# zju3dv/LoFTR

Hardware: AMD Instinct MI355X
Metric: image-pairs/sec @640x480 indoor-ds (higher is better)
Workload: dtype f32; 1 GPU; batch=8 640x480 synthetic grayscale pairs per GPU, indoor_ds dual-softmax (BASELINE configs[1]), full LoFTR.forward = ResNet-FPN backbone (HIP implicit-GEMM / patch convolutions incl. the 7x7 stem) + HIP matching path; weights=seeded random init (no checkpoint on the box), conf_matrix_materialised=True, match_type=dual_softmax, global_batch=8, parallelism=dp1 (pairs sharded; RCCL all-gather of match counts)

## Files before the change

### loftr_amd/build.py

```python
import os
import subprocess
import sys
from concurrent.futures import ThreadPoolExecutor

HERE = os.path.dirname(os.path.abspath(__file__))
CSRC = os.path.join(HERE, "csrc")
OBJ_DIR = os.path.join(CSRC, "build")
LIB_PATH = os.path.join(HERE, "libloftr_hip.so")
SOURCES = ["linear.hip", "coarse_plan.hip", "attention.hip", "transformer.hip", "coarse_match.hip", "fine.hip", "misc.hip",
           "sp_convert.hip", "conv.hip", "eval.hip", "input.hip", "comm.hip", "pose.hip", "train.hip", "train_bwd.hip", "encoder_fused.hip", "fine_fused.hip", "head_grads.hip", "encoder_bwd.hip", "fine_bwd.hip", "train_glue.hip", "bank.hip", "pose_gpu.hip", "window_head.hip", "window_head_first.hip", "geometry.hip", "geometry_gpu.hip", "absolute_pose.hip", "absolute_pose_gpu.hip", "scan.hip", "atlas.hip", "atlas_gpu.hip", "triangulate.hip", "triangulate_gpu.hip", "model_lookup.hip", "model_lookup_gpu.hip", "bundle.hip", "bundle_gpu.hip", "register.hip", "register_gpu.hip", "complete.hip", "complete_gpu.hip", "merge.hip", "merge_gpu.hip", "split.hip", "split_gpu.hip", "similarity.hip", "similarity_gpu.hip", "overlap.hip", "overlap_gpu.hip", "undistort.hip", "undistort_gpu.hip", "refine.hip", "refine_gpu.hip", "rotation.hip", "rotation_gpu.hip"]
FLAGS = ["--offload-arch=gfx950", "-O3", "-std=c++17", "-fPIC", "-Wall", "-Wno-unused-parameter"]


def _hipcc():
    for c in (os.environ.get("HIPCC"), "/opt/rocm/bin/hipcc", "hipcc"):
        if c and (os.path.isabs(c) and os.path.exists(c) or not os.path.isabs(c)):
            return c
    raise RuntimeError("hipcc not found")


def _deps_mtime():
    paths = [os.path.join(CSRC, f) for f in os.listdir(CSRC) if f.endswith((".h", ".hip"))]
    paths.append(os.path.join(os.path.dirname(HERE), "include", "loftr_hip.h"))
    return max(os.path.getmtime(p) for p in paths)


def build(force=False, verbose=True, extra_flags=(), lib_path=None, obj_dir=None):
    global LIB_PATH, OBJ_DIR
    lib_default, obj_default = LIB_PATH, OBJ_DIR
    if lib_path:
        LIB_PATH, OBJ_DIR, force = lib_path, obj_dir or (OBJ_DIR + "_variant"), True
    try:
        return _build(force, verbose, tuple(extra_flags))
    finally:
        LIB_PATH, OBJ_DIR = lib_default, obj_default


def _build(force, verbose, extra_flags):
    if not force and os.path.exists(LIB_PATH) and os.path.getmtime(LIB_PATH) >= _deps_mtime():
        return LIB_PATH
    os.makedirs(OBJ_DIR, exist_ok=True)
    hipcc = _hipcc()

    def compile_one(src):
        obj = os.path.join(OBJ_DIR, src.replace(".hip", ".o"))
        cmd = [hipcc, *FLAGS, *extra_flags, "-c", os.path.join(CSRC, src), "-o", obj]
        r = subprocess.run(cmd, capture_output=True, text=True)
        if r.returncode != 0:
            raise RuntimeError(f"hipcc failed on {src}:\n{r.stderr}")
        if verbose and r.stderr.strip():
            sys.stderr.write(r.stderr)
        return obj

    with ThreadPoolExecutor(max_workers=min(8, len(SOURCES))) as ex:
        objs = list(ex.map(compile_one, SOURCES))
    vs = os.path.join(OBJ_DIR, "exports.map")
    with open(vs, "w") as fh:
        fh.write("{ global: loftr_*; local: *; };\n")
    r = subprocess.run([hipcc, "--offload-arch=gfx950", "-shared", "-fPIC", f"-Wl,--version-script={vs}", "-o", LIB_PATH, *objs, "-ldl"],
                       capture_output=True, text=True)
    if r.returncode != 0:
        raise RuntimeError(f"link failed:\n{r.stderr}")
    if verbose:
        print(f"built {LIB_PATH} ({os.path.getsize(LIB_PATH) / 1e6:.2f} MB)")
    return LIB_PATH


if __name__ == "__main__":
    if "--variant" in sys.argv:
        i = sys.argv.index("--variant")
        name = sys.argv[i + 1]
        build(extra_flags=[a for a in sys.argv[i + 2:] if a.startswith("-")],
              lib_path=os.path.join(HERE, f"libloftr_hip_{name}.so"), obj_dir=os.path.join(CSRC, "build", f"variant_{name}"))
    else:
        build(force="--force" in sys.argv)
```

### loftr_amd/csrc/common.h

```cpp
#pragma once
#include <hip/hip_runtime.h>
#include <stdint.h>
#include <stddef.h>
#include "../../include/loftr_hip.h"

typedef float f32x16 __attribute__((ext_vector_type(16)));
typedef float f32x4 __attribute__((ext_vector_type(4)));
typedef float f32x2 __attribute__((ext_vector_type(2)));

#define LOFTR_NEG_INF (-1e9f)

#define LOFTR_CHECK_ARG(cond) do { if (!(cond)) return LOFTR_ERR_BAD_ARG; } while (0)
#define LOFTR_CHECK_LAUNCH() do { if (hipGetLastError() != hipSuccess) return LOFTR_ERR_LAUNCH; } while (0)

#ifdef __HIP_DEVICE_COMPILE__
#define LOFTR_NO_PACKED_FP32 __attribute__((target("no-packed-fp32-ops")))
#else
#define LOFTR_NO_PACKED_FP32
#endif

__host__ __device__ static inline int ceil_div(int a, int b) { return (a + b - 1) / b; }
static inline size_t align_up(size_t x, size_t a) { return (x + a - 1) / a * a; }

enum LoftrTimedKernel {
  LOFTR_T_SCORE_STATS = 0,
  LOFTR_T_SCORE_CONF = 1,
  LOFTR_T_PROJ = 2,
  LOFTR_T_LINEAR = 3,
  LOFTR_T_LINEAR_LN = 4,
  LOFTR_T_KV = 5,
  LOFTR_T_ATTN_APPLY = 6,
  LOFTR_T_ATTN_SMALL = 7,
  LOFTR_T_GATHER = 8,
  LOFTR_T_OT_STORE = 9,
  LOFTR_T_CONV = 10,
  LOFTR_T_CONV3 = 11,
  LOFTR_T_CONV3W = 12,
  LOFTR_T_ENCODER_X = 13,
  LOFTR_T_FINE_PAIR = 14,
  LOFTR_T_COUNT = 15
};
enum LoftrDebugKey {
  LOFTR_DBG_ENCODER_SCHEDULE = 0,
  LOFTR_DBG_CONV_PERSIST_CAP,
  LOFTR_DBG_WGRAD_CHUNK,
  LOFTR_DBG_REDUCE_TALL,
  LOFTR_DBG_PCT_GRID,
  LOFTR_DBG_PCT_SKIP,
  LOFTR_DBG_PCT_QUOTA,
  LOFTR_DBG_CONV_DUO,
  LOFTR_DBG_CONV_PATCH,
  LOFTR_DBG_CONV_REM,
  LOFTR_DBG_FINE_WAVES,
  LOFTR_DBG_COUNT
};
int loftr_debug_value(int key);
extern unsigned g_loftr_timing_mask;
extern int g_loftr_range_check;
void loftr_timing_mark(int id, hipStream_t st, bool end);
struct TimedLaunch {
  int id; hipStream_t st; bool on;
  TimedLaunch(int id_, hipStream_t st_) : id(id_), st(st_), on((g_loftr_timing_mask >> id_) & 1u) {
    if (on) loftr_timing_mark(id, st, false);
  }
  ~TimedLaunch() { if (on) loftr_timing_mark(id, st, true); }
};

constexpr int NUM_XCD = 8;
static inline unsigned xcd_grid(int tiles_m, int tiles_n) { return (unsigned)(NUM_XCD * ceil_div(tiles_m, NUM_XCD) * tiles_n); }
__device__ __forceinline__ bool xcd_tile(int tiles_m, int tiles_n, int& tile_m, int& tile_n) {
  const int id = blockIdx.x, xcd = id % NUM_XCD, slot = id / NUM_XCD;
  const int chunk = ceil_div(tiles_m, NUM_XCD);
  tile_n = slot % tiles_n;
  const int local = slot / tiles_n;
  tile_m = xcd * chunk + local;
  return local < chunk && tile_m < tiles_m;
}

struct WsAlloc {
  char* base; size_t cap; size_t off;
  WsAlloc(void* p, size_t bytes) : base((char*)p), cap(bytes), off(0) {}
  template <typename T> T* take(size_t n) {
    off = align_up(off, 256);
    T* r = (T*)(base + off);
    off += n * sizeof(T);
    return r;
  }
  bool ok() const { return off <= cap; }
};

__device__ __forceinline__ float wave_sum(float v) {
#pragma unroll
  for (int o = 32; o >= 1; o >>= 1) v += __shfl_xor(v, o, 64);
  return v;
}
__device__ __forceinline__ float wave_max(float v) {
#pragma unroll
  for (int o = 32; o >= 1; o >>= 1) v = fmaxf(v, __shfl_xor(v, o, 64));
  return v;
}
#define LOFTR_DPP(v_, ctrl_) __int_as_float(__builtin_amdgcn_update_dpp(0, __float_as_int(v_), ctrl_, 0xF, 0xF, true))
#define LOFTR_DPPI(v_, ctrl_) __builtin_amdgcn_update_dpp(0, v_, ctrl_, 0xF, 0xF, true)
__device__ __forceinline__ float half_sum(float v) {
  v += LOFTR_DPP(v, 0xB1);
  v += LOFTR_DPP(v, 0x4E);
  v += LOFTR_DPP(v, 0x141);
  v += LOFTR_DPP(v, 0x140);
  const auto r = __builtin_amdgcn_permlane16_swap(__float_as_int(v), __float_as_int(v), false, false);
  return __int_as_float(r[0]) + __int_as_float(r[1]);
}
__device__ __forceinline__ float half_max(float v) {
  v = fmaxf(v, LOFTR_DPP(v, 0xB1));
  v = fmaxf(v, LOFTR_DPP(v, 0x4E));
  v = fmaxf(v, LOFTR_DPP(v, 0x141));
  v = fmaxf(v, LOFTR_DPP(v, 0x140));
  const auto r = __builtin_amdgcn_permlane16_swap(__float_as_int(v), __float_as_int(v), false, false);
  return fmaxf(__int_as_float(r[0]), __int_as_float(r[1]));
}
__device__ __forceinline__ int half_min_i32(int v) {
  v = min(v, LOFTR_DPPI(v, 0xB1));
  v = min(v, LOFTR_DPPI(v, 0x4E));
  v = min(v, LOFTR_DPPI(v, 0x141));
  v = min(v, LOFTR_DPPI(v, 0x140));
  const auto r = __builtin_amdgcn_permlane16_swap(v, v, false, false);
  return min((int)r[0], (int)r[1]);
}
__device__ __forceinline__ void half_sum16(f32x16& v) {
#pragma unroll
  for (int r = 0; r < 16; ++r) v[r] += LOFTR_DPP(v[r], 0xB1);
#pragma unroll
  for (int r = 0; r < 16; ++r) v[r] += LOFTR_DPP(v[r], 0x4E);
#pragma unroll
  for (int r = 0; r < 16; ++r) v[r] += LOFTR_DPP(v[r], 0x141);
#pragma unroll
  for (int r = 0; r < 16; ++r) v[r] += LOFTR_DPP(v[r], 0x140);
#pragma unroll
  for (int r = 0; r < 16; ++r) {
    const auto q = __builtin_amdgcn_permlane16_swap(__float_as_int(v[r]), __float_as_int(v[r]), false, false);
    v[r] = __int_as_float(q[0]) + __int_as_float(q[1]);
  }
}
__device__ __forceinline__ void half_max16(f32x16& v) {
#pragma unroll
  for (int r = 0; r < 16; ++r) v[r] = fmaxf(v[r], LOFTR_DPP(v[r], 0xB1));
#pragma unroll
  for (int r = 0; r < 16; ++r) v[r] = fmaxf(v[r], LOFTR_DPP(v[r], 0x4E));
#pragma unroll
  for (int r = 0; r < 16; ++r) v[r] = fmaxf(v[r], LOFTR_DPP(v[r], 0x141));
#pragma unroll
  for (int r = 0; r < 16; ++r) v[r] = fmaxf(v[r], LOFTR_DPP(v[r], 0x140));
#pragma unroll
  for (int r = 0; r < 16; ++r) {
    const auto q = __builtin_amdgcn_permlane16_swap(__float_as_int(v[r]), __float_as_int(v[r]), false, false);
    v[r] = fmaxf(__int_as_float(q[0]), __int_as_float(q[1]));
  }
}
__device__ __forceinline__ float swap32(float v) {
  const auto r = __builtin_amdgcn_permlane32_swap(__float_as_int(v), __float_as_int(v), false, false);
  return __int_as_float((threadIdx.x & 32) ? r[0] : r[1]);
}
#define LOFTR_DPP_SWAP32(v_) swap32(v_)

__device__ __forceinline__ float elu1(float x) {
  return x > 0.f ? x + 1.f : __expf(x);
}
```

### loftr_amd/csrc/conv.hip

```cpp
#include "gemm.h"
#include "conv_prepared.h"
#include <stdlib.h>

namespace {

using CfgD = GemmCfg<256, 128, 4, 2, 3>;

struct ConvArgs {
  ASrc a;
  const sp_t* w; int K;
  const float* bias;
  const float* wscale;
  const float* x_inv;
  const sp_t* residual;
  sp_t* y_sp;
  float* y_f32;
  int M, Cout, Coutp;
  int act;
  const sp_t* up;
  int Hl, Wl;
  float sy, sx;
};

template <typename Cfg, bool FULL>
__device__ __forceinline__ void conv_epilogue(const ConvArgs& p, f32x16 (&acc)[Cfg::TM][Cfg::TN], int m0, int n0) {
  const EpiLane<Cfg> e;
  const sp_t* rs = p.residual ? p.residual + (long)m0 * p.Coutp + n0 : nullptr;
  sp_t* os = p.y_sp ? p.y_sp + (long)m0 * p.Coutp + n0 : nullptr;
  float* of = p.y_f32 ? p.y_f32 + (long)m0 * p.Cout + n0 : nullptr;
#pragma unroll
  for (int j = 0; j < Cfg::TN; ++j) {
    const int col = n0 + e.lcol + j * 32;
    const bool creal = col < p.Cout;
    const bool cpad = col < p.Coutp;
    const float b = (p.bias && creal) ? p.bias[col] : 0.f;
    const float wsc = (creal ? p.wscale[col] : 1.f) * (p.x_inv ? *p.x_inv : 1.f);
#pragma unroll
    for (int i = 0; i < Cfg::TM; ++i) {
      f32x16 v = acc[i][j] * wsc;
      if (rs) {
        uint32_t w[16];
#pragma unroll
        for (int r = 0; r < 16; ++r) {
          const int trow = e.lrow + e.rr(i, r);
          const bool ok = (FULL || m0 + trow < p.M) && cpad;
          w[r] = ok ? rs[(unsigned)(trow * p.Coutp + e.spcol + j * 32)] : 0u;
        }
#pragma unroll
        for (int r = 0; r < 16; ++r) v[r] += sp_value(w[r], e.odd);
      }
#pragma unroll
      for (int r = 0; r < 16; ++r) {
        float x = v[r] + b;
        if (p.act == 1) x = fmaxf(x, 0.f);
        if (p.act == 2) x = x > 0.f ? x : 0.01f * x;
        v[r] = creal ? x : 0.f;
      }
      if (of) {
#pragma unroll
        for (int r = 0; r < 16; ++r) {
          const int trow = e.lrow + e.rr(i, r);
          if ((FULL || m0 + trow < p.M) && creal) of[(unsigned)(trow * p.Cout + e.lcol + j * 32)] = v[r];
        }
      }
      if (os) {
        uint32_t w[16];
        sp_words16(v, e.odd, w);
#pragma unroll
        for (int r = 0; r < 16; ++r) {
          const int trow = e.lrow + e.rr(i, r);
          if ((FULL || m0 + trow < p.M) && cpad) os[(unsigned)(trow * p.Coutp + e.spcol + j * 32)] = w[r];
        }
      }
    }
  }
}

template <typename Cfg>
__device__ __forceinline__ void conv_epilogue_up(const ConvArgs& p, f32x16 (&acc)[Cfg::TM][Cfg::TN], int m0, int n0,
                                                 float* lds) {
  constexpr int LD = Cfg::BN + 4;
  static_assert(Cfg::BM * LD <= Cfg::LDS_FLOATS, "accumulator tile does not fit the operand ring");
  const EpiLane<Cfg> e;
  __syncthreads();
  const float xinv = p.x_inv ? *p.x_inv : 1.f;
#pragma unroll
  for (int j = 0; j < Cfg::TN; ++j) {
    const int col = n0 + e.lcol + j * 32;
    const float wsc = (col < p.Cout ? p.wscale[col] : 1.f) * xinv;
#pragma unroll
    for (int i = 0; i < Cfg::TM; ++i)
#pragma unroll
      for (int r = 0; r < 16; ++r) lds[(e.lrow + e.rr(i, r)) * LD + e.lcol + j * 32] = acc[i][j][r] * wsc;
  }
  __syncthreads();
  const int Wo = 2 * p.Wl, Ho = 2 * p.Hl;
  constexpr int OCTS = Cfg::BN / 8;
  for (int it = threadIdx.x; it < Cfg::BM * OCTS; it += Cfg::THREADS) {
    const int row = it / OCTS, oct = it - row * OCTS;
    const int pix = m0 + row, col0 = n0 + oct * 8;
    if (pix >= p.M || col0 >= p.Coutp) continue;
    const int t = pix / Wo, x = pix - t * Wo;
    const int bb = t / Ho, y = t - bb * Ho;
    const float fy = p.sy * (float)y, fx = p.sx * (float)x;
    const int y0 = (int)fy, x0 = (int)fx;
    const int dy = y0 < p.Hl - 1 ? p.Wl * p.Coutp : 0, dx = x0 < p.Wl - 1 ? p.Coutp : 0;
    const float ly = fy - (float)y0, lx = fx - (float)x0;
    const float hy = 1.f - ly, hx = 1.f - lx;
    const int off = sp_octet_off(col0 >> 3);
    const sp_t* s00 = p.up + (unsigned)(((bb * p.Hl + y0) * p.Wl + x0) * p.Coutp + off);
    const sp_t* src[4] = {s00, s00 + dx, s00 + dy, s00 + dy + dx};
    u32x4 hi[4], lo[4];
#pragma unroll
    for (int k = 0; k < 4; ++k) {
      hi[k] = *reinterpret_cast<const u32x4*>(src[k]);
      lo[k] = *reinterpret_cast<const u32x4*>(src[k] + 16);
    }
    float v[4][8], o[8];
#pragma unroll
    for (int k = 0; k < 4; ++k) sp_unpack8(hi[k], lo[k], v[k]);
    const f32x4 a0 = *reinterpret_cast<const f32x4*>(&lds[row * LD + oct * 8]);
    const f32x4 a1 = *reinterpret_cast<const f32x4*>(&lds[row * LD + oct * 8 + 4]);
#pragma unroll
    for (int c = 0; c < 8; ++c)
      o[c] = col0 + c < p.Cout
                 ? (c < 4 ? a0[c] : a1[c - 4]) + (hy * (hx * v[0][c] + lx * v[1][c]) + ly * (hx * v[2][c] + lx * v[3][c]))
                 : 0.f;
    u32x4 oh, ol;
    sp_pack8(o, oh, ol);
    sp_t* dst = p.y_sp + (unsigned)(pix * p.Coutp + off);
    *reinterpret_cast<u32x4*>(dst) = oh;
    *reinterpret_cast<u32x4*>(dst + 16) = ol;
  }
}

template <typename Cfg, bool UP>
__global__ __launch_bounds__(Cfg::THREADS, 2) void conv_kernel(ConvArgs p) {
  __shared__ __attribute__((aligned(16))) float lds[Cfg::LDS_FLOATS];
  int tm, tn;
  if (!xcd_tile(ceil_div(p.M, Cfg::BM), ceil_div(p.Coutp, Cfg::BN), tm, tn)) return;
  const int m0 = tm * Cfg::BM, n0 = tn * Cfg::BN;
  f32x16 acc[Cfg::TM][Cfg::TN];
  gemm_mainloop<Cfg, true>(p.a, p.w, p.K, p.M, p.Cout, p.K, m0, n0, lds, acc, p.Coutp);
  if constexpr (UP) conv_epilogue_up<Cfg>(p, acc, m0, n0, lds);
  else if (m0 + Cfg::BM <= p.M) conv_epilogue<Cfg, true>(p, acc, m0, n0);
  else conv_epilogue<Cfg, false>(p, acc, m0, n0);
}

namespace c3 {
constexpr int TY = 8, TX = 32, PW = TX + 2, PH = TY + 2, PROWS = PW * PH;
constexpr int PSLOTS = 43, PQ = 6;
constexpr int PATCH_BYTES = PSLOTS * 1024, BTILE_BYTES = 128 * 128;
constexpr int NB = 4;
constexpr int LDS_BYTES = 2 * PATCH_BYTES + NB * BTILE_BYTES + 1024;
// ... 462 lines not shown
}

template <int RT>
__global__ __launch_bounds__(256) void conv_rem_gather_kernel(const float* __restrict__ pbuf, long npix, int H, int W, int R, int c0, int Coutp,
                                                              const float* __restrict__ bias, const sp_t* __restrict__ residual, int act,
                                                              sp_t* __restrict__ y_sp) {
  const long pix = (long)blockIdx.x * 256 + threadIdx.x;
  if (pix >= npix) return;
  const int x = (int)(pix % W), y = (int)((pix / W) % H);
  float v[8];
#pragma unroll
  for (int c = 0; c < 8; ++c) v[c] = 0.f;
  const float* pp = pbuf + pix * (9 * R);
#pragma unroll
  for (int ky = 0; ky < 3; ++ky)
#pragma unroll
    for (int kx = 0; kx < 3; ++kx) {
      const int yy = y + ky - 1, xx = x + kx - 1;
      if ((unsigned)yy < (unsigned)H && (unsigned)xx < (unsigned)W) {
        const float* q = pp + ((long)(ky - 1) * W + (kx - 1)) * (9 * R) + (ky * 3 + kx) * R;
        if (RT == 4) {
          const f32x4 t = *reinterpret_cast<const f32x4*>(q);
          v[0] += t[0]; v[1] += t[1]; v[2] += t[2]; v[3] += t[3];
        } else {
#pragma unroll
          for (int c = 0; c < 7; ++c) if (c < R) v[c] += q[c];
        }
      }
    }
  sp_t* row = y_sp + pix * Coutp + c0;
  float rv[8];
#pragma unroll
  for (int c = 0; c < 8; ++c) rv[c] = 0.f;
  if (residual) {
    const sp_t* rr = residual + pix * Coutp + c0;
    const u32x4 hi = *reinterpret_cast<const u32x4*>(rr), lo = *reinterpret_cast<const u32x4*>(rr + 16);
    sp_unpack8(hi, lo, rv);
  }
  const float slope = act == 1 ? 0.f : act == 2 ? 0.01f : 1.f;
  float o[8];
#pragma unroll
  for (int c = 0; c < 8; ++c) {
    const float t = v[c] + ((bias && c < R) ? bias[c0 + c] : 0.f) + rv[c];
    o[c] = c < R ? fmaxf(t, slope * t) : 0.f;
  }
  u32x4 oh, ol;
  sp_pack8(o, oh, ol);
  const u32x4 z = {0u, 0u, 0u, 0u};
  u32x4* dst = reinterpret_cast<u32x4*>(row);
  dst[0] = oh; dst[1] = z; dst[2] = z; dst[3] = z; dst[4] = ol; dst[5] = z; dst[6] = z; dst[7] = z;
}


static int conv_prepare(const float* weight, const long* weight_strides, int Cin, int Cout, int KH, int KW,
                        const float* bn_weight, const float* bn_bias, const float* bn_mean, const float* bn_var, float bn_eps,
                        void* buf, size_t bytes, hipStream_t st) {
  LOFTR_CHECK_ARG(weight && weight_strides && buf && Cin > 0 && Cout > 0 && KH > 0 && KW > 0);
  LOFTR_CHECK_ARG((bn_weight == nullptr) == (bn_bias == nullptr) && (bn_weight == nullptr) == (bn_mean == nullptr) &&
                  (bn_weight == nullptr) == (bn_var == nullptr));
  ConvPrepared pr;
  if (!conv_prepared_layout(buf, bytes, Cin, Cout, KH, KW, pr)) return LOFTR_ERR_WORKSPACE;
  const int Cp = ceil32(Cin), K = KH * KW * Cp;
  (void)hipMemsetAsync(pr.zeros, 0, 256, st);
  hipLaunchKernelGGL(conv_rowscale_kernel, dim3(Cout), dim3(256), 0, st, weight, bn_weight, bn_bias, bn_mean, bn_var, bn_eps,
                     Cin, KH, KW, weight_strides[0], weight_strides[1], weight_strides[2], weight_strides[3], pr.bias, pr.wscale);
  hipLaunchKernelGGL(conv_prep_kernel, dim3(ceil_div(K / 32, 8), Cout), dim3(256), 0, st, weight, bn_weight, bn_bias,
                     bn_mean, bn_var, bn_eps, Cin, Cp, KH, KW, weight_strides[0], weight_strides[1], weight_strides[2],
                     weight_strides[3], pr.wsp, pr.wscale);
  LOFTR_CHECK_LAUNCH();
  return LOFTR_OK;
}

static int conv_rem_channels(int Cout, int KH, int KW, int stride) {
  return (KH == 3 && KW == 3 && stride == 1 && ceil32(Cout) == 224 && Cout - 192 >= 1 && Cout - 192 <= 7) ? Cout - 192 : 0;
}
extern "C" size_t loftr_conv_scratch_bytes(int B, int H, int W, int Cout, int KH, int KW, int stride) {
  const int R = conv_rem_channels(Cout, KH, KW, stride);
  return (R > 0 && B > 0 && H > 0 && W > 0) ? (size_t)B * H * W * 9 * R * 4 : 0;
}

static int conv_run(const uint32_t* x_sp, int B, int H, int W, int Cin, const void* prepared, size_t prepared_bytes, int Cout,
                    int KH, int KW, int stride, int pad, int act, const uint32_t* residual_sp, const uint32_t* up_sp,
                    uint32_t* y_sp, float* y_f32, void* stream, const float* x_inv = nullptr, void* scratch = nullptr, size_t scratch_bytes = 0) {
  LOFTR_CHECK_ARG(x_sp && prepared && (y_sp || y_f32) && B >= 0 && H > 0 && W > 0 && Cin > 0 && Cout > 0);
  const bool shared_gpu = (act & LOFTR_CONV_SHARED_GPU) != 0;
  act &= ~LOFTR_CONV_SHARED_GPU;
  LOFTR_CHECK_ARG(KH > 0 && KW > 0 && stride > 0 && pad >= 0 && act >= 0 && act <= 2);
  if (B == 0) return LOFTR_OK;
  hipStream_t st = (hipStream_t)stream;
  ConvGeom g;
  g.H = H; g.W = W; g.Cp = ceil32(Cin); g.KH = KH; g.KW = KW; g.stride = stride; g.pad = pad;
  g.Ho = (H + 2 * pad - KH) / stride + 1;
  g.Wo = (W + 2 * pad - KW) / stride + 1;
  if (g.Ho <= 0 || g.Wo <= 0 || H >= 32768 || W >= 32768) return LOFTR_ERR_UNSUPPORTED;
  if (up_sp && ((g.Ho & 1) || (g.Wo & 1) || KH != 1 || KW != 1 || stride != 1 || pad != 0 || !y_sp || y_f32 || residual_sp || act != 0))
    return LOFTR_ERR_UNSUPPORTED;
  const long M = (long)B * g.Ho * g.Wo;
  if (M * (long)ceil32(Cout) >= (1L << 31) || (long)B * H * W * g.Cp >= (1L << 31)) return LOFTR_ERR_UNSUPPORTED;
  const int K = KH * KW * g.Cp;
  ConvPrepared pr;
  if (!conv_prepared_layout(const_cast<void*>(prepared), prepared_bytes, Cin, Cout, KH, KW, pr)) return LOFTR_ERR_WORKSPACE;
  sp_t* wsp = pr.wsp;
  float* bias = pr.bias;
  sp_t* zeros = pr.zeros;
  g.zeros = zeros;
  ConvArgs p;
  p.a = asrc_conv(x_sp, g);
  p.w = wsp; p.K = K; p.bias = bias; p.wscale = pr.wscale; p.x_inv = x_inv; p.residual = residual_sp; p.y_sp = y_sp; p.y_f32 = y_f32;
  p.M = (int)M; p.Cout = Cout; p.Coutp = ceil32(Cout); p.act = act;
  p.up = up_sp; p.Hl = g.Ho / 2; p.Wl = g.Wo / 2;
  p.sy = g.Ho > 1 ? (float)(p.Hl - 1) / (float)(g.Ho - 1) : 0.f;
  p.sx = g.Wo > 1 ? (float)(p.Wl - 1) / (float)(g.Wo - 1) : 0.f;
  if (loftr_debug_value(LOFTR_DBG_CONV_PATCH) && KH == 3 && KW == 3 && stride == 1 && pad == 1 && !up_sp) {
    Conv3Args c;
    c.x = x_sp; c.B = B; c.H = H; c.W = W; c.Cp = g.Cp; c.Cin = Cin; c.w = wsp; c.K = K; c.bias = bias; c.wscale = pr.wscale; c.x_inv = x_inv; c.residual = residual_sp;
    c.y_sp = y_sp; c.y_f32 = y_f32; c.Cout = Cout; c.Coutp = ceil32(Cout); c.act = act; c.zeros = zeros;
    c.tiles_x = ceil_div(W, c3::TX); c.tiles_y = ceil_div(H, c3::TY); c.pbuf = nullptr;
    const bool duo = loftr_debug_value(LOFTR_DBG_CONV_DUO) != 0;
    const bool wide = duo && c.Coutp == 32 * 7;
    TimedLaunch tl(wide ? LOFTR_T_CONV3W : LOFTR_T_CONV3, st);
    if (duo && c.Coutp % 128 == 0) {
      using CF = c3d::Cfg<4, 2, 4>;
      c.tiles_y = ceil_div(H, CF::TY);
      hipLaunchKernelGGL((conv3x3_duo_kernel<CF>), dim3(xcd_grid(B * c.tiles_x * c.tiles_y, c.Coutp / 128)), dim3(256), 0, st, c);
    } else if (duo && c.Coutp == 192) {
      using CF = c3d::Cfg<6, 2, 4, 8, 2>;
      c.tiles_y = ceil_div(H, CF::TY);
      hipLaunchKernelGGL((conv3x3_duo_kernel<CF>), dim3(xcd_grid(B * c.tiles_x * c.tiles_y, 1)), dim3(512), 0, st, c);
    } else if (wide && conv_rem_channels(Cout, KH, KW, stride) > 0 && !y_f32 && loftr_debug_value(LOFTR_DBG_CONV_REM) &&
               scratch && scratch_bytes >= (size_t)B * H * W * 9 * conv_rem_channels(Cout, KH, KW, stride) * 4) {
      using CF = c3d::Cfg<6, 2, 4, 8, 2, true>;
      c.tiles_y = ceil_div(H, CF::TY);
      c.pbuf = reinterpret_cast<float*>(scratch);
      hipLaunchKernelGGL((conv3x3_duo_kernel<CF>), dim3(xcd_grid(B * c.tiles_x * c.tiles_y, 1)), dim3(512), 0, st, c);
      LOFTR_CHECK_LAUNCH();
      const long npix = (long)B * H * W;
      if (Cout - 192 == 4)
        hipLaunchKernelGGL(conv_rem_gather_kernel<4>, dim3((unsigned)((npix + 255) / 256)), dim3(256), 0, st, c.pbuf, npix, H, W, 4, 192, c.Coutp,
                           bias, residual_sp, act, y_sp);
      else
        hipLaunchKernelGGL(conv_rem_gather_kernel<0>, dim3((unsigned)((npix + 255) / 256)), dim3(256), 0, st, c.pbuf, npix, H, W, Cout - 192, 192, c.Coutp,
                           bias, residual_sp, act, y_sp);
    } else if (wide) {
      using CF = c3d::Cfg<7, 2, 4, 8, 2>;
      c.tiles_y = ceil_div(H, CF::TY);
      hipLaunchKernelGGL((conv3x3_duo_kernel<CF>), dim3(xcd_grid(B * c.tiles_x * c.tiles_y, 1)), dim3(512), 0, st, c);
    } else
      hipLaunchKernelGGL(conv3x3_kernel, dim3(shared_gpu ? xcd_grid(B * c.tiles_x * c.tiles_y, ceil_div(c.Coutp, 128))
                                                         : persistent_grid(xcd_grid(B * c.tiles_x * c.tiles_y, ceil_div(c.Coutp, 128)))),
                         dim3(512), 0, st, c);
    LOFTR_CHECK_LAUNCH();
    return LOFTR_OK;
  }
  {
    TimedLaunch tl(LOFTR_T_CONV, st);
    if (up_sp)
      hipLaunchKernelGGL((conv_kernel<CfgD, true>), dim3(xcd_grid(ceil_div(p.M, CfgD::BM), ceil_div(p.Coutp, CfgD::BN))),
                         dim3(CfgD::THREADS), 0, st, p);
    else
      hipLaunchKernelGGL((conv_kernel<CfgD, false>), dim3(xcd_grid(ceil_div(p.M, CfgD::BM), ceil_div(p.Coutp, CfgD::BN))),
                         dim3(CfgD::THREADS), 0, st, p);
  }
  LOFTR_CHECK_LAUNCH();
  return LOFTR_OK;
}

#ifdef LOFTR_CONV_PROBE
extern "C" int loftr_conv_probe_buffer(void* buf) {
  long long* b = (long long*)buf;
  return hipMemcpyToSymbol(HIP_SYMBOL(g_conv_probe), &b, sizeof(b)) == hipSuccess ? LOFTR_OK : LOFTR_ERR_LAUNCH;
}
#endif

extern "C" int loftr_conv_prepare(const float* weight, const long* weight_strides, int Cin, int Cout, int KH, int KW,
                                  const float* bn_weight, const float* bn_bias, const float* bn_mean, const float* bn_var,
                                  float bn_eps, void* prepared, size_t prepared_bytes, void* stream) {
  return conv_prepare(weight, weight_strides, Cin, Cout, KH, KW, bn_weight, bn_bias, bn_mean, bn_var, bn_eps, prepared,
                      prepared_bytes, (hipStream_t)stream);
}

extern "C" int loftr_conv_bn_act_prepared(const uint32_t* x_sp, int B, int H, int W, int Cin, const void* prepared,
                                          size_t prepared_bytes, int Cout, int KH, int KW, int stride, int pad, int act,
                                          const uint32_t* residual_sp, const uint32_t* low_sp, uint32_t* y_sp, float* y_f32,
                                          const float* x_inv_scale, void* stream) {
  return conv_run(x_sp, B, H, W, Cin, prepared, prepared_bytes, Cout, KH, KW, stride, pad, act, residual_sp, low_sp, y_sp, y_f32,
                  stream, x_inv_scale);
}

extern "C" int loftr_conv_bn_act_prepared_scratch(const uint32_t* x_sp, int B, int H, int W, int Cin, const void* prepared,
                                                  size_t prepared_bytes, int Cout, int KH, int KW, int stride, int pad, int act,
                                                  const uint32_t* residual_sp, const uint32_t* low_sp, uint32_t* y_sp, float* y_f32,
                                                  const float* x_inv_scale, void* scratch, size_t scratch_bytes, void* stream) {
  return conv_run(x_sp, B, H, W, Cin, prepared, prepared_bytes, Cout, KH, KW, stride, pad, act, residual_sp, low_sp, y_sp, y_f32,
                  stream, x_inv_scale, scratch, scratch_bytes);
}

extern "C" int loftr_conv_bn_act(const uint32_t* x_sp, int B, int H, int W, int Cin, const float* weight,
                                 const long* weight_strides, int Cout, int KH, int KW, int stride, int pad, const float* bn_weight, const float* bn_bias,
                                 const float* bn_mean, const float* bn_var, float bn_eps, int act,
                                 const uint32_t* residual_sp, uint32_t* y_sp, float* y_f32, void* ws, size_t ws_bytes,
                                 const float* x_inv_scale, void* stream) {
  LOFTR_CHECK_ARG(x_sp && (y_sp || y_f32) && B >= 0 && H > 0 && W > 0);
  if (B == 0) return LOFTR_OK;
  const int rc = conv_prepare(weight, weight_strides, Cin, Cout, KH, KW, bn_weight, bn_bias, bn_mean, bn_var, bn_eps, ws, ws_bytes,
                              (hipStream_t)stream);
  if (rc != LOFTR_OK) return rc;
  return conv_run(x_sp, B, H, W, Cin, ws, ws_bytes, Cout, KH, KW, stride, pad, act, residual_sp, nullptr, y_sp, y_f32, stream, x_inv_scale);
}

extern "C" int loftr_conv1x1_upsample_add(const uint32_t* x_sp, int B, int H, int W, int Cin, const float* weight,
                                          const long* weight_strides, int Cout, const uint32_t* low_sp, uint32_t* y_sp,
                                          void* ws, size_t ws_bytes, void* stream) {
  LOFTR_CHECK_ARG(x_sp && low_sp && y_sp && B >= 0 && H > 0 && W > 0);
  if (B == 0) return LOFTR_OK;
  const int rc = conv_prepare(weight, weight_strides, Cin, Cout, 1, 1, nullptr, nullptr, nullptr, nullptr, 0.f, ws, ws_bytes,
                              (hipStream_t)stream);
  if (rc != LOFTR_OK) return rc;
  return conv_run(x_sp, B, H, W, Cin, ws, ws_bytes, Cout, 1, 1, 1, 0, 0, nullptr, low_sp, y_sp, nullptr, stream);
}

extern "C" int loftr_stem_conv_bn_relu(const float* x, const long* x_strides, int B, int H, int W, const float* weight,
                                       const long* weight_strides, int C0, const float* bn_weight, const float* bn_bias,
                                       const float* bn_mean, const float* bn_var, float bn_eps, uint32_t* y_sp,
                                       void* stream) {
  LOFTR_CHECK_ARG(x && x_strides && weight && weight_strides && y_sp && B >= 0 && H > 0 && W > 0 && C0 > 0);
  LOFTR_CHECK_ARG((bn_weight == nullptr) == (bn_bias == nullptr) && (bn_weight == nullptr) == (bn_mean == nullptr) &&
                  (bn_weight == nullptr) == (bn_var == nullptr));
  if (C0 > 128) return LOFTR_ERR_UNSUPPORTED;
  if (B == 0) return LOFTR_OK;
  const int Ho = (H + 6 - 7) / 2 + 1, Wo = (W + 6 - 7) / 2 + 1;
  hipLaunchKernelGGL(stem_conv_kernel, dim3(ceil_div(Wo, STEM_TX), ceil_div(Ho, STEM_TY), B), dim3(256), 0,
                     (hipStream_t)stream, x, x_strides[0], x_strides[2], x_strides[3], H, W, weight, weight_strides[0],
                     weight_strides[2], weight_strides[3], bn_weight, bn_bias, bn_mean, bn_var, bn_eps, C0, Ho, Wo, y_sp);
  LOFTR_CHECK_LAUNCH();
  return LOFTR_OK;
}

extern "C" int loftr_upsample2x_add(const uint32_t* low_sp, const uint32_t* lateral_sp, uint32_t* out_sp, int B, int Hl,
                                    int Wl, int C, void* stream) {
  LOFTR_CHECK_ARG(low_sp && lateral_sp && out_sp && B >= 0 && Hl > 0 && Wl > 0 && C > 0);
  if (B == 0) return LOFTR_OK;
  const int Cp = ceil32(C);
  const long pixels = (long)B * 4 * Hl * Wl;
  if (pixels >= (1L << 31)) return LOFTR_ERR_UNSUPPORTED;
  const long nitems = pixels * (Cp / 8);
  if ((nitems + 255) / 256 >= (1L << 31)) return LOFTR_ERR_UNSUPPORTED;
  hipLaunchKernelGGL(upsample_add_kernel, dim3((unsigned)((nitems + 255) / 256)), dim3(256), 0, (hipStream_t)stream,
                     low_sp, lateral_sp, out_sp, Hl, Wl, Cp, nitems);
  LOFTR_CHECK_LAUNCH();
  return LOFTR_OK;
}

extern "C" int loftr_sp_from_f32(const float* src, uint32_t* dst_sp, long rows, int C, void* stream) {
  LOFTR_CHECK_ARG(src && dst_sp && rows >= 0 && C > 0);
  return launch_sp_convert1(src, C, dst_sp, rows, C, (hipStream_t)stream);
}

extern "C" int loftr_sp_from_f32_scaled(const float* src, uint32_t* dst_sp, long rows, int C, float* inv_scale_out, void* stream) {
  LOFTR_CHECK_ARG(src && dst_sp && inv_scale_out && rows >= 0 && C > 0);
  return launch_sp_convert1(src, C, dst_sp, rows, C, (hipStream_t)stream, inv_scale_out);
}

extern "C" int loftr_sp_to_f32(const uint32_t* src_sp, float* dst, long rows, int C, void* stream) {
  LOFTR_CHECK_ARG(src_sp && dst && rows >= 0 && C > 0);
  if (rows == 0) return LOFTR_OK;
  const int Cp = ceil32(C);
  hipLaunchKernelGGL(sp_to_f32_kernel, dim3((unsigned)rows), dim3(Cp > 256 ? 256 : Cp), 0, (hipStream_t)stream, src_sp,
                     dst, rows, C, Cp);
  LOFTR_CHECK_LAUNCH();
  return LOFTR_OK;
}
```

### loftr_amd/csrc/misc.hip

```cpp
#include "common.h"
#include <string.h>

namespace {
template <bool CL>
__global__ void pos_encode_flatten_kernel(loftr_fmap f, const float* __restrict__ pe,
                                          int pe_h, int pe_w, float* __restrict__ out, int C) {
  __shared__ float tile[32][33];
  const int H = f.H, W = f.W, HW = H * W;
  const int n = blockIdx.z, hw0 = blockIdx.x * 32, c0 = blockIdx.y * 32;
  const float* in = f.data + (long)n * f.sn;
  for (int k = threadIdx.y; k < 32; k += 8) {
    const int c = c0 + k, hw = hw0 + threadIdx.x;
    float v = 0.f;
    if (c < C && hw < HW) {
      const int y = hw / W, x = hw - y * W;
      v = pe[((long)c * pe_h + y) * pe_w + x];
      if (!CL) v += in[(long)c * f.sc + (long)y * f.sh + (long)x * f.sw];
    }
    tile[k][threadIdx.x] = v;
  }
  __syncthreads();
  for (int k = threadIdx.y; k < 32; k += 8) {
    const int hw = hw0 + k, c = c0 + threadIdx.x;
    if (hw < HW && c < C) {
      float v = tile[threadIdx.x][k];
      if (CL) { const int y = hw / W, x = hw - y * W; v += in[(long)y * f.sh + (long)x * f.sw + c]; }
      out[((long)n * HW + hw) * C + c] = v;
    }
  }
}
}

extern "C" int loftr_pos_encode_flatten(const loftr_fmap* feat, const float* pe, int pe_h, int pe_w, float* out,
                                        int N, int C, void* stream) {
  LOFTR_CHECK_ARG(feat && feat->data && pe && out && N >= 0 && C > 0 && feat->H > 0 && feat->W > 0 &&
                  feat->H <= pe_h && feat->W <= pe_w);
  if (N == 0) return LOFTR_OK;
  const dim3 grid(ceil_div(feat->H * feat->W, 32), ceil_div(C, 32), N), block(32, 8);
  if (feat->sc == 1)
    hipLaunchKernelGGL((pos_encode_flatten_kernel<true>), grid, block, 0, (hipStream_t)stream, *feat, pe, pe_h, pe_w, out, C);
  else
    hipLaunchKernelGGL((pos_encode_flatten_kernel<false>), grid, block, 0, (hipStream_t)stream, *feat, pe, pe_h, pe_w, out, C);
  LOFTR_CHECK_LAUNCH();
  return LOFTR_OK;
}

namespace {
struct DebugSwitch { const char* name; int def; int value; };
DebugSwitch g_debug[LOFTR_DBG_COUNT] = {{"encoder_schedule", 1, 1}, {"conv_persist_cap", 0, 0}, {"wgrad_chunk", 0, 0}, {"reduce_tall", 1, 1},
                                        {"pct_grid", 0, 0}, {"pct_skip", 0, 0}, {"pct_quota", 0, 0}, {"conv_duo", 1, 1}, {"conv_patch", 1, 1}, {"conv_rem", 1, 1},
                                        {"fine_waves", 0, 0}};
}
int loftr_debug_value(int key) { return (key >= 0 && key < LOFTR_DBG_COUNT) ? g_debug[key].value : 0; }
extern "C" int loftr_hip_debug_set(const char* key, int value) {
  LOFTR_CHECK_ARG(key != nullptr);
  for (auto& d : g_debug)
    if (strcmp(d.name, key) == 0) { d.value = value; return LOFTR_OK; }
  return LOFTR_ERR_BAD_ARG;
}
extern "C" int loftr_hip_debug_get(const char* key, int* value, int* default_value) {
  LOFTR_CHECK_ARG(key != nullptr && value != nullptr);
  for (auto& d : g_debug)
    if (strcmp(d.name, key) == 0) { *value = d.value; if (default_value) *default_value = d.def; return LOFTR_OK; }
  return LOFTR_ERR_BAD_ARG;
}

unsigned g_loftr_timing_mask = 0;
int g_loftr_range_check = 0;
extern "C" int loftr_hip_range_check_enable(int on) { g_loftr_range_check = on ? 1 : 0; return LOFTR_OK; }
namespace {
constexpr int T_POOL = 4096;
struct TimingSlot {
  hipEvent_t ev[T_POOL][2];
  int created, used;
  double total_ms; long long launches;
};
TimingSlot g_slots[LOFTR_T_COUNT];
const char* const T_NAMES[LOFTR_T_COUNT] = {"score_sweep_kernel<0>", "score_sweep_kernel<1>", "proj_kernel", "linear_kernel",
                                            "linear_ln_kernel", "proj_kv_kernel", "attn_apply_kernel",
                                            "attn_small_kernel", "gather_windows_kernel", "score_sweep_kernel<2>", "conv_kernel",
                                            "conv3x3_duo_kernel<Cfg<4,2,4,4,1>>", "conv3x3_duo_kernel<Cfg<7,2,4,8,2>>", "encoder_x_kernel", "fine_pair_kernel"};
void timing_drain(TimingSlot& s) {
  for (int i = 0; i < s.used; ++i) {
    float ms = 0.f;
    if (hipEventSynchronize(s.ev[i][1]) == hipSuccess && hipEventElapsedTime(&ms, s.ev[i][0], s.ev[i][1]) == hipSuccess) {
      s.total_ms += ms;
      s.launches += 1;
    }
  }
  s.used = 0;
}
}

void loftr_timing_mark(int id, hipStream_t st, bool end) {
  TimingSlot& s = g_slots[id];
  if (!end) {
    if (s.used >= T_POOL) return;
    if (s.used >= s.created) {
      if (hipEventCreate(&s.ev[s.created][0]) != hipSuccess || hipEventCreate(&s.ev[s.created][1]) != hipSuccess) return;
      s.created++;
    }
    (void)hipEventRecord(s.ev[s.used][0], st);
  } else {
    if (s.used >= s.created) return;
    (void)hipEventRecord(s.ev[s.used][1], st);
    s.used++;
  }
}

extern "C" int loftr_hip_timing_enable(unsigned mask) {
  g_loftr_timing_mask = mask & ((1u << LOFTR_T_COUNT) - 1u);
  return LOFTR_OK;
}

extern "C" int loftr_hip_timing_kernel_count(void) { return LOFTR_T_COUNT; }

extern "C" const char* loftr_hip_timing_kernel_name(int id) {
  return (id >= 0 && id < LOFTR_T_COUNT) ? T_NAMES[id] : "";
}

extern "C" int loftr_hip_timing_read(int id, double* total_ms, long long* launches, int reset) {
  LOFTR_CHECK_ARG(id >= 0 && id < LOFTR_T_COUNT && total_ms && launches);
  TimingSlot& s = g_slots[id];
  timing_drain(s);
  *total_ms = s.total_ms;
  *launches = s.launches;
  if (reset) { s.total_ms = 0.0; s.launches = 0; }
  return LOFTR_OK;
}

extern "C" int loftr_hip_abi_version(void) { return LOFTR_HIP_ABI_VERSION; }

extern "C" const char* loftr_hip_status_string(int status) {
  switch (status) {
    case LOFTR_OK: return "ok";
    case LOFTR_ERR_BAD_ARG: return "bad argument (null pointer or invalid shape)";
    case LOFTR_ERR_UNSUPPORTED: return "shape not supported by the gfx950 kernels";
    case LOFTR_ERR_WORKSPACE: return "workspace too small";
    case LOFTR_ERR_LAUNCH: return "HIP kernel launch failed";
    case LOFTR_ERR_NO_DEVICE: return "no gfx950 (MI355X) device";
    case LOFTR_ERR_COMM: return "RCCL unavailable or a communicator / collective call failed";
    case LOFTR_ERR_RANGE: return "an activation entering the split-fp16 GEMM chain is not below the fp16 maximum 65504 (or not finite)";
    default: return "unknown status";
  }
}

extern "C" int loftr_hip_device_check(void) {
  int dev = 0;
  if (hipGetDevice(&dev) != hipSuccess) return LOFTR_ERR_NO_DEVICE;
  hipDeviceProp_t prop;
  if (hipGetDeviceProperties(&prop, dev) != hipSuccess) return LOFTR_ERR_NO_DEVICE;
  return strncmp(prop.gcnArchName, "gfx950", 6) == 0 ? LOFTR_OK : LOFTR_ERR_NO_DEVICE;
}
```

Measured before the change: 478.0 image-pairs/s.

## Add pipelined split-fp16 MFMA implicit-GEMM conv path for 224-channel layers

Adds a new implicit-GEMM convolution kernel that streams activation patches and weights into LDS through direct global-to-LDS loads with a multi-stage pipeline, then runs split-fp16 32x32x16 MFMAs with pinned scheduling. It is enabled by default for convolutions without upsample or residual inputs, but the default rule only selects it for Coutp==224, choosing a wide or lean tile form depending on kernel size. It aims to replace the generic conv kernel for those layers with better overlap of loads and math, at the cost of more code paths and tuning that may not suit every shape.

```diff
diff --git a/loftr_amd/build.py b/loftr_amd/build.py
--- a/loftr_amd/build.py
+++ b/loftr_amd/build.py
@@ -8,7 +8,7 @@
 OBJ_DIR = os.path.join(CSRC, "build")
 LIB_PATH = os.path.join(HERE, "libloftr_hip.so")
 SOURCES = ["linear.hip", "coarse_plan.hip", "attention.hip", "transformer.hip", "coarse_match.hip", "fine.hip", "misc.hip",
-           "sp_convert.hip", "conv.hip", "eval.hip", "input.hip", "comm.hip", "pose.hip", "train.hip", "train_bwd.hip", "encoder_fused.hip", "fine_fused.hip", "head_grads.hip", "encoder_bwd.hip", "fine_bwd.hip", "train_glue.hip", "bank.hip", "pose_gpu.hip", "window_head.hip", "window_head_first.hip", "geometry.hip", "geometry_gpu.hip", "absolute_pose.hip", "absolute_pose_gpu.hip", "scan.hip", "atlas.hip", "atlas_gpu.hip", "triangulate.hip", "triangulate_gpu.hip", "model_lookup.hip", "model_lookup_gpu.hip", "bundle.hip", "bundle_gpu.hip", "register.hip", "register_gpu.hip", "complete.hip", "complete_gpu.hip", "merge.hip", "merge_gpu.hip", "split.hip", "split_gpu.hip", "similarity.hip", "similarity_gpu.hip", "overlap.hip", "overlap_gpu.hip", "undistort.hip", "undistort_gpu.hip", "refine.hip", "refine_gpu.hip", "rotation.hip", "rotation_gpu.hip"]
+           "sp_convert.hip", "conv.hip", "entry_gemm.hip", "eval.hip", "input.hip", "comm.hip", "pose.hip", "train.hip", "train_bwd.hip", "encoder_fused.hip", "fine_fused.hip", "head_grads.hip", "encoder_bwd.hip", "fine_bwd.hip", "train_glue.hip", "bank.hip", "pose_gpu.hip", "window_head.hip", "window_head_first.hip", "geometry.hip", "geometry_gpu.hip", "absolute_pose.hip", "absolute_pose_gpu.hip", "scan.hip", "atlas.hip", "atlas_gpu.hip", "triangulate.hip", "triangulate_gpu.hip", "model_lookup.hip", "model_lookup_gpu.hip", "bundle.hip", "bundle_gpu.hip", "register.hip", "register_gpu.hip", "complete.hip", "complete_gpu.hip", "merge.hip", "merge_gpu.hip", "split.hip", "split_gpu.hip", "similarity.hip", "similarity_gpu.hip", "overlap.hip", "overlap_gpu.hip", "undistort.hip", "undistort_gpu.hip", "refine.hip", "refine_gpu.hip", "rotation.hip", "rotation_gpu.hip"]
 FLAGS = ["--offload-arch=gfx950", "-O3", "-std=c++17", "-fPIC", "-Wall", "-Wno-unused-parameter"]
 
 
diff --git a/loftr_amd/csrc/common.h b/loftr_amd/csrc/common.h
--- a/loftr_amd/csrc/common.h
+++ b/loftr_amd/csrc/common.h
@@ -52,6 +52,7 @@
   LOFTR_DBG_CONV_PATCH,
   LOFTR_DBG_CONV_REM,
   LOFTR_DBG_FINE_WAVES,
+  LOFTR_DBG_CONV_ENTRY,
   LOFTR_DBG_COUNT
 };
 int loftr_debug_value(int key);
diff --git a/loftr_amd/csrc/conv.hip b/loftr_amd/csrc/conv.hip
--- a/loftr_amd/csrc/conv.hip
+++ b/loftr_amd/csrc/conv.hip
@@ -1,5 +1,6 @@
 #include "gemm.h"
 #include "conv_prepared.h"
+#include "entry_gemm.h"
 #include <stdlib.h>
 
 namespace {
@@ -768,6 +769,21 @@
     LOFTR_CHECK_LAUNCH();
     return LOFTR_OK;
   }
+  const int entry = loftr_debug_value(LOFTR_DBG_CONV_ENTRY);
+  if (entry && !up_sp && !residual_sp && egm::entry_gemm_takes(p.Coutp)) {
+    egm::Args e;
+    e.x = x_sp; e.H = H; e.W = W; e.Cp = g.Cp; e.Cin = Cin; e.KH = KH; e.KW = KW; e.stride = stride; e.pad = pad; e.Ho = g.Ho; e.Wo = g.Wo;
+    e.zeros = zeros; e.w = wsp; e.K = K; e.bias = bias; e.wscale = pr.wscale; e.x_inv = x_inv; e.y_sp = y_sp; e.y_f32 = y_f32;
+    e.M = p.M; e.Cout = Cout; e.Coutp = p.Coutp; e.act = act;
+    const egm::Form form = entry == 2 ? egm::FORM_LEAN : entry == 3 ? egm::FORM_WIDE : egm::entry_gemm_rule(e);
+    if (form != egm::FORM_NONE) {
+      TimedLaunch tl(LOFTR_T_CONV, st);
+      const int rc = egm::launch_entry_gemm(e, form, st);
+      if (rc != LOFTR_OK) return rc;
+      LOFTR_CHECK_LAUNCH();
+      return LOFTR_OK;
+    }
+  }
   {
     TimedLaunch tl(LOFTR_T_CONV, st);
     if (up_sp)
diff --git a/loftr_amd/csrc/entry_gemm.h b/loftr_amd/csrc/entry_gemm.h
--- /dev/null
+++ b/loftr_amd/csrc/entry_gemm.h
@@ -0,0 +1,18 @@
+#pragma once
+#include "gemm.h"
+
+namespace egm {
+struct Args {
+  const sp_t* x; int H, W, Cp, Cin;
+  int KH, KW, stride, pad, Ho, Wo;
+  const sp_t* zeros;
+  const sp_t* w; int K;
+  const float* bias; const float* wscale; const float* x_inv;
+  sp_t* y_sp; float* y_f32;
+  int M, Cout, Coutp, act;
+};
+enum Form { FORM_NONE = 0, FORM_LEAN = 1, FORM_WIDE = 2 };
+bool entry_gemm_takes(int Coutp);
+Form entry_gemm_rule(const Args& a);
+int launch_entry_gemm(const Args& a, Form form, hipStream_t st);
+}
diff --git a/loftr_amd/csrc/entry_gemm.hip b/loftr_amd/csrc/entry_gemm.hip
--- /dev/null
+++ b/loftr_amd/csrc/entry_gemm.hip
@@ -0,0 +1,290 @@
+#include "entry_gemm.h"
+
+#ifndef EGM_SETPRIO
+#define EGM_SETPRIO 0
+#endif
+#ifndef EGM_PIN
+#define EGM_PIN 1
+#endif
+
+namespace egm {
+
+template <int NT_, int RW_, int WAVES_, int WN_, int NB_>
+struct Cfg {
+  static constexpr int NT = NT_, RW = RW_, WAVES = WAVES_, WN = WN_, NB = NB_, LA = NB_ - 1;
+  static constexpr int WM = WAVES / WN, NJ = (NT + WN - 1) / WN;
+  static constexpr int BM = WM * RW * 32;
+  static constexpr int ASLOTS = BM / 16, AQ = ASLOTS / WAVES;
+  static constexpr int BSLOTS = NT * 2, BQ = (BSLOTS + WAVES - 1) / WAVES;
+  static constexpr int PER = AQ + BQ;
+  static constexpr int STAGE_BYTES = (ASLOTS + BSLOTS) * 1024;
+  static constexpr int LDS_BYTES = NB * STAGE_BYTES + 1024;
+  static constexpr int WG_PER_CU = WAVES == 4 ? 2 : 1;
+  static_assert(ASLOTS % WAVES == 0, "A slots divide evenly over the waves");
+  static_assert(LDS_BYTES * WG_PER_CU <= 160 * 1024, "LDS");
+  static_assert(RW * NJ <= 8, "128 accumulator registers");
+  static_assert(LA >= 2 && LA <= 3, "vmcnt bookkeeping below");
+  static_assert(NT - (WN - 1) * NJ >= 1, "every column split owns a tile");
+};
+
+template <int J, int NJW, int RW>
+__device__ __forceinline__ void pin_tiles() {
+  if constexpr (J + 1 < NJW) {
+    __builtin_amdgcn_sched_group_barrier(0x008, 1, 0);
+    __builtin_amdgcn_sched_group_barrier(0x100, 1, 0);
+    __builtin_amdgcn_sched_group_barrier(0x008, 1, 0);
+    __builtin_amdgcn_sched_group_barrier(0x100, 1, 0);
+    __builtin_amdgcn_sched_group_barrier(0x008, 3 * RW - 2, 0);
+    pin_tiles<J + 1, NJW, RW>();
+  } else {
+    __builtin_amdgcn_sched_group_barrier(0x008, 3 * RW, 0);
+  }
+}
+
+struct StepPos {
+  int ky, kx, q;
+  int aoff;
+  int boff;
+};
+
+template <typename CF, int NJW>
+__device__ __forceinline__ void k_loop(const Args& p, char* lds, char* scratch, const int (&aoff)[CF::AQ], const int (&ayx)[CF::AQ],
+                                       const int (&boff)[CF::BQ], int nhalf, int ns, int wave, const int (&abase)[CF::RW],
+                                       const int (&bbase)[CF::NJ], f32x16 (&acc)[CF::RW][CF::NJ]) {
+  constexpr int RW = CF::RW, NB = CF::NB, LA = CF::LA, AQ = CF::AQ, BQ = CF::BQ, WAVES = CF::WAVES, PER = CF::PER;
+  typedef __attribute__((address_space(3))) void* lds_ptr_t;
+  typedef const __attribute__((address_space(1))) void* gbl_ptr_t;
+  StepPos ip = {0, 0, 0, 0, 0};
+#define EGM_ISSUE(stage_)                                                                                   \
+  {                                                                                                         \
+    const sp_t* xb__ = p.x;                                                                                 \
+    const sp_t* wb__ = p.w;                                                                                 \
+    asm volatile("" : "+s"(xb__), "+s"(wb__));                                                              \
+    char* dst__ = lds + (stage_) * CF::STAGE_BYTES;                                                         \
+    const int ko__ = (ip.q >> 1) * 32 + (ip.q & 1) * 8;                                                     \
+    _Pragma("unroll") for (int q = 0; q < AQ; ++q) {                                                        \
+      const int y__ = (ayx[q] >> 16) + ip.ky, x__ = (int)(short)(ayx[q] & 0xffff) + ip.kx;                  \
+      const bool in__ = (unsigned)y__ < (unsigned)p.H && (unsigned)x__ < (unsigned)p.W;                     \
+      const sp_t* g__ = in__ ? xb__ + (aoff[q] + ip.aoff + ko__) : p.zeros;                                 \
+      __builtin_amdgcn_global_load_lds((gbl_ptr_t)g__, (lds_ptr_t)(dst__ + (q * WAVES + wave) * 1024), 16, 0, 0); \
+    }                                                                                                       \
+    _Pragma("unroll") for (int q = 0; q < BQ; ++q) {                                                        \
+      const bool used__ = q * WAVES + wave < CF::BSLOTS;                                  \
+      const sp_t* g__ = used__ ? wb__ + (boff[q] + ip.boff + ko__) : p.zeros;                               \
+      char* d__ = used__ ? dst__ + (CF::ASLOTS + q * WAVES + wave) * 1024 : scratch;                        \
+      __builtin_amdgcn_global_load_lds((gbl_ptr_t)g__, (lds_ptr_t)d__, 16, 0, 0);                           \
+    }                                                                                                       \
+    if (++ip.q == nhalf) {                                                                                  \
+      ip.q = 0;                                                                                             \
+      ip.aoff += p.Cp; ip.boff += p.Cp;                                                                     \
+      if (++ip.kx == p.KW) { ip.kx = 0; ++ip.ky; ip.aoff += (p.W - p.KW) * p.Cp; }                          \
+    }                                                                                                       \
+  }
+#pragma unroll
+  for (int s = 0; s < LA; ++s)
+    if (s < ns) EGM_ISSUE(s);
+  int stage = 0;
+  for (int s = 0; s < ns; ++s) {
+    const int newer = min(LA - 1, ns - 1 - s);
+    if (LA == 3 && newer >= 2) LOFTR_WAITCNT_VM(2 * PER);
+    else if (newer >= 1) LOFTR_WAITCNT_VM(PER);
+    else LOFTR_WAITCNT_VM(0);
+    __builtin_amdgcn_s_barrier();
+    if (s + LA < ns) EGM_ISSUE(stage + LA >= NB ? stage + LA - NB : stage + LA);
+    const char* sA = lds + stage * CF::STAGE_BYTES;
+    const char* sB = sA + CF::ASLOTS * 1024;
+    h16x8 ah[RW], al[RW];
+#pragma unroll
+    for (int i = 0; i < RW; ++i) {
+      ah[i] = *reinterpret_cast<const h16x8*>(sA + abase[i]);
+      al[i] = *reinterpret_cast<const h16x8*>(sA + (abase[i] ^ 32));
+    }
+    h16x8 ch = *reinterpret_cast<const h16x8*>(sB + bbase[0]);
+    h16x8 cl = *reinterpret_cast<const h16x8*>(sB + (bbase[0] ^ 32));
+#pragma unroll
+    for (int j = 0; j < NJW; ++j) {
+      h16x8 nh = ch, nl = cl;
+      if (j + 1 < NJW) {
+        nh = *reinterpret_cast<const h16x8*>(sB + bbase[j + 1 < CF::NJ ? j + 1 : 0]);
+        nl = *reinterpret_cast<const h16x8*>(sB + (bbase[j + 1 < CF::NJ ? j + 1 : 0] ^ 32));
+      }
+#pragma unroll
+      for (int i = 0; i < RW; ++i) acc[i][j] = __builtin_amdgcn_mfma_f32_32x32x16_f16(al[i], ch, acc[i][j], 0, 0, 0);
+#pragma unroll
+      for (int i = 0; i < RW; ++i) acc[i][j] = __builtin_amdgcn_mfma_f32_32x32x16_f16(ah[i], cl, acc[i][j], 0, 0, 0);
+#pragma unroll
+      for (int i = 0; i < RW; ++i) acc[i][j] = __builtin_amdgcn_mfma_f32_32x32x16_f16(ah[i], ch, acc[i][j], 0, 0, 0);
+      ch = nh; cl = nl;
+    }
+    if (EGM_PIN) {
+      __builtin_amdgcn_sched_group_barrier(0x100, 2 * RW + 2, 0);
+      pin_tiles<0, NJW, RW>();
+    }
+    stage = stage + 1 == NB ? 0 : stage + 1;
+  }
+#undef EGM_ISSUE
+}
+
+template <typename CF>
+__global__ __launch_bounds__(CF::WAVES * 64, CF::WG_PER_CU) void entry_gemm_kernel(Args p) {
+  constexpr int NT = CF::NT, RW = CF::RW, NB = CF::NB, AQ = CF::AQ, BQ = CF::BQ, WAVES = CF::WAVES, WM = CF::WM, NJ = CF::NJ, BM = CF::BM;
+  __shared__ __attribute__((aligned(16))) char lds[CF::LDS_BYTES];
+  char* const scratch = lds + NB * CF::STAGE_BYTES;
+  int tm, tn;
+  if (!xcd_tile(ceil_div(p.M, BM), 1, tm, tn)) return;
+  const int m0 = tm * BM;
+
+  const int tid = threadIdx.x, lane = tid & 63, wave = tid >> 6;
+  const int g = lane >> 5, tx = lane & 31;
+  const int wr = wave % WM, wn = wave / WM;
+  const int jc0 = wn * NJ;
+  const int nj = min(NJ, NT - jc0);
+  const int drow = lane >> 2, dpos = lane & 3;
+
+  int aoff[AQ], ayx[AQ], boff[BQ];
+#pragma unroll
+  for (int q = 0; q < AQ; ++q) {
+    const int r = (q * WAVES + wave) * 16 + drow;
+    const int c = dpos ^ ((r >> 2) & 3);
+    const int gr = min(m0 + r, p.M - 1);
+    const int hw = p.Ho * p.Wo;
+    const int b = gr / hw, rem = gr - b * hw;
+    const int yo = rem / p.Wo, xo = rem - yo * p.Wo;
+    const int yb = yo * p.stride - p.pad, xb = xo * p.stride - p.pad;
+    ayx[q] = (yb << 16) | (xb & 0xffff);
+    aoff[q] = ((b * p.H + yb) * p.W + xb) * p.Cp + (((c & 1) + ((c >> 1) << 2)) << 2);
+  }
+#pragma unroll
+  for (int q = 0; q < BQ; ++q) {
+    const int r = (q * WAVES + wave) * 16 + drow;
+    const int c = dpos ^ ((r >> 2) & 3);
+    boff[q] = min(r, p.Cout - 1) * p.K + (((c & 1) + ((c >> 1) << 2)) << 2);
+  }
+  const int gpt = p.Cp >> 5;
+  const int nhalf = 2 * gpt - (p.Cin <= (gpt - 1) * 32 + 16 ? 1 : 0), ns = nhalf * p.KH * p.KW;
+
+  int abase[RW], bbase[NJ];
+#pragma unroll
+  for (int i = 0; i < RW; ++i) {
+    const int ar = (wr * RW + i) * 32 + tx;
+    abase[i] = ar * 64 + ((g ^ ((ar >> 2) & 3)) << 4);
+  }
+#pragma unroll
+  for (int j = 0; j < NJ; ++j) {
+    const int br = min(jc0 + j, NT - 1) * 32 + tx;
+    bbase[j] = br * 64 + ((g ^ ((br >> 2) & 3)) << 4);
+  }
+  f32x16 acc[RW][NJ];
+#pragma unroll
+  for (int i = 0; i < RW; ++i)
+#pragma unroll
+    for (int j = 0; j < NJ; ++j)
+#pragma unroll
+      for (int r = 0; r < 16; ++r) acc[i][j][r] = 0.f;
+
+  if (EGM_SETPRIO) __builtin_amdgcn_s_setprio(1);
+  if (CF::WN == 1 || nj == NJ) k_loop<CF, NJ>(p, lds, scratch, aoff, ayx, boff, nhalf, ns, wave, abase, bbase, acc);
+  else k_loop<CF, (NJ > 1 ? NJ - 1 : 1)>(p, lds, scratch, aoff, ayx, boff, nhalf, ns, wave, abase, bbase, acc);
+
+  if (EGM_SETPRIO) __builtin_amdgcn_s_setprio(0);
+  const bool odd = lane & 1;
+  const float xinv = p.x_inv ? *p.x_inv : 1.f;
+  const int mw = m0 + wr * RW * 32;
+  if (m0 + BM <= p.M) {
+    const unsigned lane_sp = (unsigned)(4 * g * p.Coutp + (odd ? 16 : 0) + (tx >> 1));
+    const unsigned lane_f32 = (unsigned)(4 * g * p.Cout + tx);
+#pragma unroll
+    for (int j = 0; j < NJ; ++j) {
+      if (j >= nj) continue;
+      const int col = (jc0 + j) * 32 + tx;
+      const bool creal = col < p.Cout;
+      const float b = (p.bias && creal) ? p.bias[col] : 0.f;
+      const float wsc = (creal ? p.wscale[col] : 1.f) * xinv;
+#pragma unroll
+      for (int i = 0; i < RW; ++i) {
+        f32x16 v = acc[i][j] * wsc;
+#pragma unroll
+        for (int r = 0; r < 16; ++r) {
+          float x = v[r] + b;
+          if (p.act == 1) x = fmaxf(x, 0.f);
+          if (p.act == 2) x = x > 0.f ? x : 0.01f * x;
+          v[r] = creal ? x : 0.f;
+        }
+        if (p.y_f32 && creal) {
+          float* op = p.y_f32 + ((size_t)(mw + i * 32) * p.Cout + (jc0 + j) * 32);
+#pragma unroll
+          for (int r = 0; r < 16; ++r) (op + (size_t)(((r & 3) + 8 * (r >> 2)) * p.Cout))[lane_f32] = v[r];
+        }
+        if (p.y_sp) {
+          uint32_t w16[16];
+          sp_words16(v, odd, w16);
+          sp_t* op = p.y_sp + ((size_t)(mw + i * 32) * p.Coutp + (jc0 + j) * 32);
+#pragma unroll
+          for (int r = 0; r < 16; ++r) (op + (size_t)(((r & 3) + 8 * (r >> 2)) * p.Coutp))[lane_sp] = w16[r];
+        }
+      }
+    }
+  } else {
+#pragma unroll
+    for (int j = 0; j < NJ; ++j) {
+      if (j >= nj) continue;
+      const int col = (jc0 + j) * 32 + tx;
+      const bool creal = col < p.Cout;
+      const float b = (p.bias && creal) ? p.bias[col] : 0.f;
+      const float wsc = (creal ? p.wscale[col] : 1.f) * xinv;
+      const int spc = (col & ~31) + (odd ? 16 : 0) + ((col & 31) >> 1);
+#pragma unroll
+      for (int i = 0; i < RW; ++i) {
+        f32x16 v = acc[i][j] * wsc;
+#pragma unroll
+        for (int r = 0; r < 16; ++r) {
+          float x = v[r] + b;
+          if (p.act == 1) x = fmaxf(x, 0.f);
+          if (p.act == 2) x = x > 0.f ? x : 0.01f * x;
+          v[r] = creal ? x : 0.f;
+        }
+        if (p.y_f32) {
+#pragma unroll
+          for (int r = 0; r < 16; ++r) {
+            const int row = mw + i * 32 + (r & 3) + 8 * (r >> 2) + 4 * g;
+            if (row < p.M && creal) p.y_f32[(size_t)row * p.Cout + col] = v[r];
+          }
+        }
+        if (p.y_sp) {
+          uint32_t w16[16];
+          sp_words16(v, odd, w16);
+#pragma unroll
+          for (int r = 0; r < 16; ++r) {
+            const int row = mw + i * 32 + (r & 3) + 8 * (r >> 2) + 4 * g;
+            if (row < p.M) p.y_sp[(size_t)row * p.Coutp + spc] = w16[r];
+          }
+        }
+      }
+    }
+  }
+}
+
+template <typename CF>
+static void launch(const Args& a, hipStream_t st) {
+  hipLaunchKernelGGL((entry_gemm_kernel<CF>), dim3(xcd_grid(ceil_div(a.M, CF::BM), 1)), dim3(CF::WAVES * 64), 0, st, a);
+}
+
+bool entry_gemm_takes(int Coutp) { return Coutp == 128 || Coutp == 224 || Coutp == 256; }
+
+Form entry_gemm_rule(const Args& a) {
+  if (a.Coutp == 224) return a.KH * a.KW > 1 ? FORM_WIDE : FORM_LEAN;
+  return FORM_NONE;
+}
+
+int launch_entry_gemm(const Args& a, Form form, hipStream_t st) {
+  const bool wide = form == FORM_WIDE;
+  switch (a.Coutp) {
+    case 128: launch<Cfg<4, 2, 4, 1, 3>>(a, st); break;
+    case 224: if (wide) launch<Cfg<7, 2, 8, 2, 4>>(a, st); else launch<Cfg<7, 1, 4, 1, 3>>(a, st); break;
+    case 256: if (wide) launch<Cfg<8, 2, 8, 2, 4>>(a, st); else launch<Cfg<8, 1, 4, 1, 3>>(a, st); break;
+    default: return LOFTR_ERR_UNSUPPORTED;
+  }
+  return LOFTR_OK;
+}
+
+}
diff --git a/loftr_amd/csrc/misc.hip b/loftr_amd/csrc/misc.hip
--- a/loftr_amd/csrc/misc.hip
+++ b/loftr_amd/csrc/misc.hip
@@ -49,7 +49,7 @@
 struct DebugSwitch { const char* name; int def; int value; };
 DebugSwitch g_debug[LOFTR_DBG_COUNT] = {{"encoder_schedule", 1, 1}, {"conv_persist_cap", 0, 0}, {"wgrad_chunk", 0, 0}, {"reduce_tall", 1, 1},
                                         {"pct_grid", 0, 0}, {"pct_skip", 0, 0}, {"pct_quota", 0, 0}, {"conv_duo", 1, 1}, {"conv_patch", 1, 1}, {"conv_rem", 1, 1},
-                                        {"fine_waves", 0, 0}};
+                                        {"fine_waves", 0, 0}, {"conv_entry", 1, 1}};
 }
 int loftr_debug_value(int key) { return (key >= 0 && key < LOFTR_DBG_COUNT) ? g_debug[key].value : 0; }
 extern "C" int loftr_hip_debug_set(const char* key, int value) {
```

After: 474.9 image-pairs/s. No clear change (-0.7%).
